# wei-zeng98/piano-a2s

Measured on AMD Instinct MI355X. Metric: training clips/sec (12 s, 5-bar), higher is better.
Workload: dtype f32

## Files before the change

include/a2s.h:

```cpp
#ifndef A2S_H
#define A2S_H
#include <stddef.h>
#include <stdint.h>
#ifdef __cplusplus
extern "C" {
#endif

#define A2S_OK 0
#define A2S_ERR_ARG (-1)
#define A2S_ERR_HIP (-2)
#define A2S_ERR_WORKSPACE (-3)

const char* a2s_last_error(void);
int a2s_version(void);
long long a2s_launch_count(void);

int a2s_gemm_f32(void* stream, int M, int N, int K, float alpha, const float* A, long sAm, long sAk,
                 const float* B, long sBk, long sBn, float beta, float* C, long ldc, const float* bias, int act,
                 int batch, long bsA, long bsB, long bsC, int splitk, float* workspace, size_t workspace_bytes);
int a2s_gemm_f32_affine(void* stream, int M, int N, int K, float alpha, const float* A, long sAm, long sAk, const float* B, long sBk,
                        long sBn, float beta, float* C, long ldc, const float* bias, int act, int batch, long bsA, long bsB, long bsC,
                        int splitk, float* workspace, size_t workspace_bytes, const float* a_scale, const float* a_shift, int a_period,
                        const float* b_scale, const float* b_shift, int b_period);
int a2s_gemm_f32_bnstats(void* stream, int M, int N, int K, const float* A, long sAm, long sAk, const float* B, long sBk, long sBn, float* C, long ldc,
// ... 7 lines not shown
                                const float* a_absmax, const float* b_absmax);
int a2s_linear_dgrad_bnstats(void* stream, int M, int N, int K, const float* dz, long lda, const float* Wt, float* da, long ldc, const float* y,
                             const float* mean, const float* invstd, const float* scale, const float* shift, int period, float* partial,
                             const float* dz_absmax, const float* w_absmax, float* workspace, size_t workspace_bytes, float* da_absmax_out);
int a2s_linear_fwd(void* stream, int M, int N, int K, const float* y, long lda, const float* W, float* z, long ldc, const float* scale, const float* shift,
                   int period, const float* y_absmax, const float* w_absmax, float* workspace, size_t workspace_bytes);
int a2s_linear_fwd_eligible(int M, int N, int K, int period);
int a2s_linear_wgrad(void* stream, int M, int N, int K, const float* dz, long ldz, const float* y, long lda, float* G, long ldg, const float* scale,
                     const float* shift, int period, const float* dz_absmax, const float* y_absmax, float* workspace, size_t workspace_bytes);
size_t a2s_linear_wgrad_ws_bytes(int M, int K);
int a2s_linear_wgrad_eligible(int M, int N, int K, int period);
int a2s_tallk_wgrad(void* stream, int M, int Np, int K, const float* P, long ldp, const float* A, long lda, float* G, long ldg, int transposed, float* bias,
                    const float* p_absmax, const float* a_absmax, float* workspace, size_t workspace_bytes);
size_t a2s_tallk_wgrad_ws_bytes(int M, int Np, int K);
int a2s_tallk_wgrad_eligible(int M, int Np, int K, long ldp, long lda, long ldg, int transposed);
size_t a2s_linear_dgrad_ws_bytes(int N, int K);
int a2s_linear_dgrad_blocks(int M);
int a2s_linear_dgrad_eligible(int M, int N, int K, int period);
int a2s_absmax(void* stream, const float* x, long n, float* out);
int a2s_gemm_bnstats_blocks(int M, int period);
size_t a2s_gemm_workspace_bytes(int M, int N, int batch, int splitk);
int a2s_gemm_pick_splitk(int M, int N, int K, int batch);
void a2s_gemm_debug_tile(int cfg);
int a2s_debug_set(const char* key, int value);
int a2s_debug_get(const char* key);
int a2s_env_check(void);
int a2s_persist_abort_latch(void* device_word);

int a2s_conv3x3(void* stream, const float* x, const float* w, float* y, const float* in_scale, const float* in_shift,
                float* stat_partial, int B, int T, int F, int Cin, int Cout, int flip, float* workspace);
// ... 323 lines not shown
```

piano_a2s_amd/csrc/a2s_api.hip:

```cpp
#define A2S_SWITCHES_IMPL
#include "a2s_internal.h"

thread_local char a2s_err_msg[512] = {0};
long long a2s_launch_counter = 0;

#define ST ((hipStream_t)stream)

extern "C" {

const char* a2s_last_error(void) { return a2s_err_msg; }
int a2s_version(void) { return 1; }
long long a2s_launch_count(void) { return __atomic_load_n(&a2s_launch_counter, __ATOMIC_RELAXED); }

int a2s_gemm_f32(void* stream, int M, int N, int K, float alpha, const float* A, long sAm, long sAk, const float* B, long sBk,
                 long sBn, float beta, float* C, long ldc, const float* bias, int act, int batch, long bsA, long bsB, long bsC,
                 int splitk, float* workspace, size_t workspace_bytes) {
    return a2s_gemm_impl(ST, M, N, K, alpha, A, sAm, sAk, B, sBk, sBn, beta, C, ldc, bias, act, batch, bsA, bsB, bsC, splitk,
                         workspace, workspace_bytes);
}
int a2s_gemm_f32_affine(void* stream, int M, int N, int K, float alpha, const float* A, long sAm, long sAk, const float* B, long sBk,
                        long sBn, float beta, float* C, long ldc, const float* bias, int act, int batch, long bsA, long bsB, long bsC,
                        int splitk, float* workspace, size_t workspace_bytes, const float* a_scale, const float* a_shift, int a_period,
                        const float* b_scale, const float* b_shift, int b_period) {
    return a2s_gemm_affine_impl(ST, M, N, K, alpha, A, sAm, sAk, B, sBk, sBn, beta, C, ldc, bias, act, batch, bsA, bsB, bsC, splitk,
// ... 27 lines not shown
    return a2s_linear_fwd_impl(ST, M, N, K, y, lda, W, z, ldc, scale, shift, period, y_absmax, w_absmax, workspace, workspace_bytes);
}
int a2s_linear_wgrad(void* stream, int M, int N, int K, const float* dz, long ldz, const float* y, long lda, float* G, long ldg, const float* scale,
                     const float* shift, int period, const float* dz_absmax, const float* y_absmax, float* workspace, size_t workspace_bytes) {
    return a2s_linear_wgrad_impl(ST, M, N, K, dz, ldz, y, lda, G, ldg, scale, shift, period, dz_absmax, y_absmax, workspace, workspace_bytes);
}
size_t a2s_linear_wgrad_ws_bytes(int M, int K) { return a2s_linear_wgrad_ws_bytes_impl(M, K); }
int a2s_linear_wgrad_eligible(int M, int N, int K, int period) { return a2s_linear_wgrad_ok(M, N, K, 256, 4, 4, period, nullptr, nullptr, nullptr) ? 1 : 0; }
int a2s_tallk_wgrad(void* stream, int M, int Np, int K, const float* P, long ldp, const float* A, long lda, float* G, long ldg, int transposed, float* bias,
                    const float* p_absmax, const float* a_absmax, float* workspace, size_t workspace_bytes) {
    return a2s_tallk_wgrad_impl(ST, M, Np, K, P, ldp, A, lda, G, ldg, transposed, bias, p_absmax, a_absmax, workspace, workspace_bytes);
}
size_t a2s_tallk_wgrad_ws_bytes(int M, int Np, int K) { return a2s_tallk_wgrad_ws_bytes_impl(M, Np, K); }
int a2s_tallk_wgrad_eligible(int M, int Np, int K, long ldp, long lda, long ldg, int transposed) {
    return a2s_tallk_wgrad_ok(M, Np, K, ldp, lda, ldg, transposed, nullptr, nullptr, nullptr, nullptr) ? 1 : 0;
}
int a2s_linear_fwd_eligible(int M, int N, int K, int period) { return a2s_linear_fwd_ok(M, N, K, 4, 4, period, nullptr, nullptr, nullptr) ? 1 : 0; }
int a2s_linear_dgrad_blocks(int M) { return a2s_linear_dgrad_blocks_impl(M); }
int a2s_linear_dgrad_eligible(int M, int N, int K, int period) {
    return a2s_linear_dgrad_ok(M, N, K, 4, 1, K, 4, period, nullptr, nullptr, nullptr, nullptr) ? 1 : 0;
}
int a2s_gemm_f32_bnstats(void* stream, int M, int N, int K, const float* A, long sAm, long sAk, const float* B, long sBk, long sBn, float* C, long ldc,
                         const float* y, const float* mean, const float* invstd, const float* scale, const float* shift, int period, float* partial) {
    return a2s_gemm_affine_impl(ST, M, N, K, 1.f, A, sAm, sAk, B, sBk, sBn, 0.f, C, ldc, nullptr, 0, 1, 0, 0, 0, 1, nullptr, 0,
                                nullptr, nullptr, 0, nullptr, nullptr, 0, y, mean, invstd, scale, shift, partial, period, 0, nullptr, nullptr);
}
int a2s_gemm_bnstats_blocks(int M, int period) { return a2s_cdiv(M, 128) * a2s_gemm_bnstats_slots(period); }
size_t a2s_gemm_workspace_bytes(int M, int N, int batch, int splitk) { return a2s_gemm_workspace_bytes_impl(M, N, batch, splitk); }
int a2s_gemm_pick_splitk(int M, int N, int K, int batch) { return a2s_gemm_pick_splitk_impl(M, N, K, batch); }
void a2s_gemm_debug_tile(int cfg) { a2s_gemm_debug_tile_impl(cfg); }
size_t a2s_note_step_workspace_floats(int H, int E) { return a2s_note_step_workspace_floats_impl(H, E); }
int a2s_debug_set(const char* key, int value) {
    if (!key) return A2S_ERR_ARG;
    const int id = a2s_switch_find(key);
    if (id >= 0) { a2s_switch_store(id, value); return A2S_OK; }
    if (!strcmp(key, "attn_deferred_fast")) { a2s_attn_deferred_fast = value ? 1 : 0; return A2S_OK; }
    if (!strcmp(key, "tallk_wgrad")) { a2s_tallk_wgrad_on = value ? 1 : 0; return A2S_OK; }
    if (!strcmp(key, "tallk_wgrad_max_splits")) { a2s_tallk_wgrad_max_splits = value > 0 ? value : 0; return A2S_OK; }
    if (!strcmp(key, "gemm_tile")) { a2s_gemm_debug_tile_impl(value); return A2S_OK; }
    snprintf(a2s_err_msg, sizeof(a2s_err_msg), "a2s_debug_set: unknown key %s", key);
    return A2S_ERR_ARG;
}
int a2s_env_check(void) {
    if (const char* e = a2s_switch_env_error()) A2S_FAIL(A2S_ERR_ARG, "%s: expected a decimal number >= 0", e);
    return A2S_OK;
}

int a2s_persist_abort_latch(void* device_word) { a2s_persist_latch_set(device_word); return A2S_OK; }

int a2s_debug_get(const char* key) {
    if (!key) return -1;
    const int id = a2s_switch_find(key);
    if (id == A2S_SW_attn_pair_fused_rows) return a2s_attn_pair_fused_rows();
    if (id >= 0) return a2s_sw((a2s_switch)id);
    if (!strcmp(key, "attn_pair_launches")) return (int)a2s_attn_pair_launches();
    if (!strcmp(key, "attn_pair_bwd_launches")) return (int)a2s_attn_pair_bwd_launches();
    if (!strcmp(key, "attn_deferred_fast")) return a2s_attn_deferred_fast;
    if (!strcmp(key, "tallk_wgrad")) return a2s_tallk_wgrad_on;
    if (!strcmp(key, "tallk_wgrad_max_splits")) return a2s_tallk_wgrad_max_splits;
    if (!strcmp(key, "tallk_wgrad_launches")) return (int)a2s_tallk_wgrad_launches();
    if (!strcmp(key, "attn_dk_ahead_launches")) return (int)a2s_attn_dk_ahead_launches();
    if (!strcmp(key, "attn_denc_launches")) return (int)a2s_attn_denc_launches();
    if (!strcmp(key, "dec_mid_launches")) return a2s_dec_mid_launches();
    if (!strcmp(key, "dec_cmb_launches")) return a2s_dec_cmb_launches();
    if (!strcmp(key, "dec_persist_launches")) return a2s_dec_persist_launches();
    if (!strcmp(key, "edit_distance_launches")) return (int)a2s_edit_distance_launches();
    if (!strcmp(key, "conv_rows16_c20_launches")) return (int)a2s_conv_rows16_c20_launches();
    if (!strcmp(key, "device_cus")) return a2s_device_geometry().cus;
    if (!strcmp(key, "device_xccs")) return a2s_device_geometry().xccs;
    return -1;
}

int a2s_conv3x3(void* stream, const float* x, const float* w, float* y, const float* in_scale, const float* in_shift,
                float* stat_partial, int B, int T, int F, int Cin, int Cout, int flip, float* workspace) {
    return a2s_conv3x3_impl(ST, x, w, y, in_scale, in_shift, stat_partial, B, T, F, Cin, Cout, flip, workspace, nullptr, nullptr, nullptr, nullptr, nullptr, nullptr,
// ... 411 lines not shown
```

piano_a2s_amd/csrc/a2s_bwd.hip:

```cpp
#include "a2s_internal.h"

__global__ __launch_bounds__(256) void log_softmax_bwd_rows(const float* __restrict__ g, const float* __restrict__ y,
                                                            long outer_stride, int inner, float* __restrict__ dx,
                                                            int R, int V, int n_outer, int time_major) {
    const int row = blockIdx.x * 4 + (threadIdx.x >> 6), lane = threadIdx.x & 63;
    if (row >= R) return;
    const int ob = row / inner, in = row % inner;
    const float* gr = g + (long)ob * outer_stride + (long)in * V;
    const float* yr = y + (long)ob * outer_stride + (long)in * V;
    float s = 0.f;
    for (int j = lane; j < V; j += 64) s += gr[j];
    s = wave_sum(s);
    const long orow = time_major ? ((long)in * n_outer + ob) : row;
    for (int j = lane; j < V; j += 64) dx[orow * V + j] = gr[j] - expf(yr[j]) * s;
}

int a2s_log_softmax_bwd_rows_impl(hipStream_t st, const float* g, const float* y, long outer_stride, int inner, float* dx,
                                  int R, int V, int n_outer, int time_major) {
    hipLaunchKernelGGL(log_softmax_bwd_rows, dim3(a2s_cdiv(R, 4)), dim3(256), 0, st, g, y, outer_stride, inner, dx, R, V, n_outer, time_major);
    A2S_CHECK_LAUNCH("log_softmax_bwd_rows");
    return A2S_OK;
}

__global__ void gru_gates_bwd(const float* __restrict__ dh_a, long lda, const float* __restrict__ dh_b, long ldb,
// ... 540 lines not shown
    if (idx >= rows * cols) return;
    const int c = idx / rows, r = idx % rows;
    out[idx] = in[(long)r * cols + c];
}

int a2s_gru_seq_bwd_impl(hipStream_t st, const float* dout, long do_bstride, long do_tstride, const float* out, long out_bstride,
                         long out_tstride, const float* gates, const float* w_hh, const float* dhn, float* dgi_all, float* dgh_shift,
                         float* dgh_first, float* dhbuf, float* dgh_tmp, int B, int T, int H, int reverse, float* ws, size_t ws_bytes,
                         float* ranges_out, int* ranges_valid) {
    A2S_REQUIRE(dout && out && gates && w_hh && dgi_all && dgh_shift && dgh_first && dhbuf && dgh_tmp, "gru_seq_bwd: null tensor");
    if (ranges_valid) *ranges_valid = 0;
    hipError_t e;
    if (dhn) e = hipMemcpyAsync(dhbuf, dhn, sizeof(float) * B * H, hipMemcpyDeviceToDevice, st);
    else e = hipMemsetAsync(dhbuf, 0, sizeof(float) * B * H, st);
    if (e != hipSuccess) A2S_FAIL(A2S_ERR_HIP, "gru_seq_bwd init: %s", hipGetErrorString(e));
    e = hipMemsetAsync(dgh_shift, 0, sizeof(float) * (size_t)B * T * 3 * H, st);
    if (e != hipSuccess) A2S_FAIL(A2S_ERR_HIP, "gru_seq_bwd memset: %s", hipGetErrorString(e));
    const bool fused = a2s_sw(A2S_SW_gru_fused) && H % 32 == 0 && ws && ws_bytes >= sizeof(float) * 3 * H * H && ((uintptr_t)ws % 16 == 0);
    if (fused) {
        hipLaunchKernelGGL(transpose_f32, dim3(a2s_cdiv(3 * H * H, 256)), dim3(256), 0, st, w_hh, ws, 3 * H, H);
        A2S_CHECK_LAUNCH("transpose_f32");
    }
    if (fused && a2s_gru_seq_bwd_persist_ok(B, T, H, ws, ws_bytes, sizeof(float) * 3 * (size_t)H * H)) {
        const int rc = a2s_gru_seq_bwd_persist_impl(st, dout, do_bstride, do_tstride, out, out_bstride, out_tstride, gates, ws, dhn, dgi_all, dgh_shift, dgh_first,
                                                    B, T, H, reverse, ws, sizeof(float) * 3 * (size_t)H * H, ws_bytes, ranges_out);
        if (rc == A2S_OK && ranges_out && ranges_valid) *ranges_valid = 1;
        return rc;
    }
    if (fused && ws_bytes >= sizeof(float) * (3 * (size_t)H * H + 3 * (size_t)B * H) && (3 * H * H) % 4 == 0) {
        float* tmp[2] = {dgh_tmp, ws + 3 * (size_t)H * H};
        auto tix = [&](int s) { return reverse ? T - 1 - s : s; };
// ... 895 lines not shown
```

piano_a2s_amd/csrc/a2s_internal.h:

```cpp
#pragma once
#include "a2s_common.h"
#include "../../include/a2s.h"
#include "a2s_switches.h"

static inline int a2s_attn_pair_fused_rows(void) {
    const int cap = a2s_sw(A2S_SW_dec_fused_max_rows), v = a2s_sw(A2S_SW_attn_pair_fused_rows);
    return v < cap ? v : cap;
}
static inline unsigned a2s_persist_dbg(void) {
    return (a2s_sw(A2S_SW_persist_force_agent) ? PERSIST_DBG_FORCE_AGENT : 0u) | (a2s_sw(A2S_SW_persist_inject_abort) ? PERSIST_DBG_INJECT_ABORT : 0u);
}

int a2s_absmax_impl(hipStream_t st, const float* x, long n, float* out);
size_t a2s_gemm_workspace_bytes_impl(int M, int N, int batch, int splitk);
int a2s_gemm_pick_splitk_impl(int M, int N, int K, int batch);
int a2s_gemm_bnstats_slots(int period);
void a2s_gemm_debug_tile_impl(int cfg);
int a2s_gemm_affine_impl(hipStream_t st, int M, int N, int K, float alpha, const float* A, long sAm, long sAk,
    const float* B, long sBk, long sBn, float beta, float* C, long ldc, const float* bias, int act,
    int batch, long bsA, long bsB, long bsC, int splitk, float* ws, size_t ws_bytes,
    const float* a_scale, const float* a_shift, int a_period, const float* b_scale, const float* b_shift, int b_period,
    const float* ep_y, const float* ep_mean, const float* ep_invstd, const float* ep_scale, const float* ep_shift,
    float* ep_partial, int ep_period, int two_term, const float* a_absmax, const float* b_absmax);
int a2s_gemm_impl(hipStream_t st, int M, int N, int K, float alpha, const float* A, long sAm, long sAk,
// ... 8 lines not shown
    float* partial, const float* a_absmax, const float* b_absmax, float* ws, size_t ws_bytes, float* c_absmax_out);
bool a2s_linear_fwd_ok(int M, int N, int K, long lda, long ldc, int period, const void* A, const void* W, const void* C);
int a2s_linear_fwd_impl(hipStream_t st, int M, int N, int K, const float* A, long lda, const float* W, float* C, long ldc, const float* a_scale,
    const float* a_shift, int period, const float* a_absmax, const float* w_absmax, float* ws, size_t ws_bytes);
size_t a2s_linear_wgrad_ws_bytes_impl(int M, int K);
bool a2s_linear_wgrad_ok(int M, int N, int K, long ldz, long lda, long ldg, int period, const void* dz, const void* A, const void* G);
int a2s_linear_wgrad_impl(hipStream_t st, int M, int N, int K, const float* dz, long ldz, const float* A, long lda, float* G, long ldg, const float* a_scale,
    const float* a_shift, int period, const float* dz_absmax, const float* a_absmax, float* ws, size_t ws_bytes);
extern int a2s_tallk_wgrad_on;
extern int a2s_tallk_wgrad_max_splits;
long a2s_tallk_wgrad_launches(void);
size_t a2s_tallk_wgrad_ws_bytes_impl(int M, int Np, int K);
bool a2s_tallk_wgrad_ok(int M, int Np, int K, long ldp, long lda, long ldg, int transposed, const void* P, const void* A, const void* G, const void* bias);
int a2s_tallk_wgrad_impl(hipStream_t st, int M, int Np, int K, const float* P, long ldp, const float* A, long lda, float* G, long ldg, int transposed,
    float* bias, const float* p_absmax, const float* a_absmax, float* ws, size_t ws_bytes);

int a2s_act_bound_impl(hipStream_t st, const float* scale, const float* shift, const float* absmax, int C, float* out);
size_t a2s_conv3x3_workspace_floats_impl(int Cin);
int a2s_conv3x3_impl(hipStream_t st, const float* x, const float* w, float* y, const float* in_scale,
    const float* in_shift, float* stat_partial, int B, int T, int F, int Cin, int Cout, int flip, float* ws,
    const float* yl, const float* yl_mean, const float* yl_invstd, const float* yl_scale, const float* yl_shift,
    const float* x_absmax, const float* in_absmax, float* out_absmax);
int a2s_conv3x3_stat_blocks_impl(int B, int T, int F, int Cin);
int a2s_bn_finalize_impl(hipStream_t st, const float* partial, int nblocks, int C, double count, const float* gamma,
    const float* beta, float* running_mean, float* running_var, long long* nbt, float* mean,
    float* invstd, float* scale, float* shift, float eps, float momentum, int training);
int a2s_bn_relu_apply_impl(hipStream_t st, const float* x, float* y, const float* scale, const float* shift, long n, int C, int F);
int a2s_col_stats_impl(hipStream_t st, const float* x, float* partial, long rows, int C, int rows_per_block);
int a2s_bn1d_relu_dropout_impl(hipStream_t st, const float* x, float* y, const float* scale, const float* shift,
    const uint8_t* mask, float inv_keep, long n, int C);
// ... 325 lines not shown
```

piano_a2s_amd/csrc/a2s_linear.hip:

```cpp
#include "a2s_internal.h"

#define LIN_BM 128
#define LIN_K 256
#define LIN_RS 288
#define LIN_NTH 512
#define LIN_LDS (2 * 2 * LIN_BM * LIN_RS)

typedef unsigned lu32x4 __attribute__((ext_vector_type(4)));

struct LinDgradArgs {
    const float* A; long lda;
    const unsigned char* planes;
    float* C; long ldc;
    const float* ep_y;
    const float* mean; const float* invstd; const float* scale; const float* shift;
    float* partial;
    const float* a_absmax; const float* b_absmax;
    int M, N, period, channels;
    float* c_absmax_out;
};

__global__ __launch_bounds__(256) void lin_pack_planes_k(const float* __restrict__ W, long ld, int N, int K, const float* __restrict__ absmax,
                                                         unsigned char* __restrict__ out) {
    const long id = (long)blockIdx.x * 256 + threadIdx.x;
// ... 646 lines not shown
    hipLaunchKernelGGL(lin_pack_dz_planes, dim3((unsigned)(((long)nsteps * 1024 + 255) / 256), npb), dim3(256), 0, st, P, ldp, M, nsteps, p_absmax, planes);
    A2S_CHECK_LAUNCH("lin_pack_dz_planes");
    LinWgradArgs a{A, lda, planes, partial, nullptr, nullptr, a_absmax, p_absmax, M, K, K, nblk, (nblk + splits - 1) / splits, (long)plane_stride, Np,
                   bias ? bias_partial : nullptr};
    if (bias) hipLaunchKernelGGL(lin_wgrad_roles<true>, dim3(K / LIN_BM, splits, npb), dim3(LIN_NTH), 0, st, a);
    else hipLaunchKernelGGL(lin_wgrad_roles<false>, dim3(K / LIN_BM, splits, npb), dim3(LIN_NTH), 0, st, a);
    A2S_CHECK_LAUNCH("lin_wgrad (tall-K)");
    const long n = (long)Np * K, nthreads = (n + (bias ? K : 0)) / 4;
    const dim3 rgrid((unsigned)((nthreads + 255) / 256));
    if (transposed) hipLaunchKernelGGL(lin_wgrad_reduce<true>, rgrid, dim3(256), 0, st, partial, splits, n, G, ldg, K, bias ? bias_partial : nullptr, bias);
    else hipLaunchKernelGGL(lin_wgrad_reduce<false>, rgrid, dim3(256), 0, st, partial, splits, n, G, ldg, K, bias ? bias_partial : nullptr, bias);
    A2S_CHECK_LAUNCH("lin_wgrad_reduce");
    __atomic_fetch_add(&g_tallk_launches, 1LL, __ATOMIC_RELAXED);
    return A2S_OK;
}
```

piano_a2s_amd/engine_bwd.py:

```python
import ctypes as C
import os
import threading
from collections import namedtuple

import torch

from . import hip
from .conv_bwd_plan import CHANS, ConvBwdFlags, plan_convstack_bwd
from .dec_bwd_plan import dim, plan_note_decoder_bwd, plan_staff_issue
from .spec import SOS, VOCAB_SIZE


def _ptr(t, off=0):
    return C.c_void_p(t.data_ptr() + 4 * off)


_COLSUM_WS = {}


def _colsum(x, ld, out, rows, ncol, x_off=0, out_off=0, beta=1.0):
    ws = None
    if rows >= 2048:
        key = (x.device, torch.cuda.current_stream().cuda_stream, threading.get_ident())
        ws = _COLSUM_WS.get(key)
# ... 362 lines not shown
            wg = _weight_grad_stream(dev)
            wg.wait_stream(torch.cuda.current_stream())
            with torch.cuda.stream(wg):
                for fn, ev, tensors in self.late:
                    wg.wait_event(ev)
                    for t in tensors:
                        if t is not None:
                            t.record_stream(wg)
                    fn()
            late_join = dec_lo
            self.late = []
        else:
            for gf in self.group_flat[1:]:
                flat.add_(gf)
        d_hid_carry = self.d_hidden
        if self.concurrent:
            dEnc.add_(self.dEnc_staff[0]).add_(self.dEnc_staff[1])
        enc2d = enc.view(B * T, H2)
        enc_amax = hip.absmax(enc)
        for p, dKp in dK.items():
            Wn = p + ".attn.attn.weight"
            dk_amax = hip.absmax(dKp)
            if not hip.tallk_wgrad(dKp, 0, H, enc2d, 0, H2, G[Wn], H2, 4 * H, B * T, H, H2, dk_amax, enc_amax):
                sk = L.a2s_gemm_pick_splitk(H, H2, B * T, 1)
                hip.gemm(dKp, 1, H, enc2d, H2, 1, G[Wn], 4 * H, H, H2, B * T, beta=1.0, splitk=sk, c_off=H2, two_term=(dk_amax, enc_amax))
            hip.gemm(dKp, H, 1, S[Wn], 4 * H, 1, dEnc, H2, B * T, H2, H, beta=1.0, b_off=H2, two_term=(dk_amax, hip.absmax(S[Wn])))
        if late_join is not None:
            wg = _weight_grad_stream(dev)
            wg.wait_stream(torch.cuda.current_stream())
            with torch.cuda.stream(wg):
                for gf in self.group_flat[1:]:
                    flat[late_join:].add_(gf[late_join:])
                if Backward.check_fold:
                    for gi, gf in enumerate(self.group_flat[1:], 1):
                        assert not bool(gf[:late_join].any()), f"clip group {gi}: non-decoder gradients in the group buffer would be lost by the late fold"
        d_conv = _encoder_bwd(eng, S, G, sv["enc"], dEnc, d_hid_carry, B, T)
        n_conv = next(off for k, off in zip(names, offs) if not k.startswith("convstack."))
        if grad_ready is not None:
            with torch.cuda.stream(_weight_grad_stream(dev)):
                grad_ready(self.flat_full, n_conv, total + 1)
        if getattr(eng, "conv_unperm", None) is not None:
# ... 71 lines not shown
            dgh_first, dhbuf, dgh_tmp = torch.empty((B, 3 * H), device=dev), torch.empty((2, B, H), device=dev), torch.empty((B, 3 * H), device=dev)
            ranges, valid = torch.empty(2, device=dev), C.c_int(0)
            if L.a2s_debug_get(b"tallk_wgrad") > 0:
                hip.check(L.a2s_gru_seq_bwd_ranged(hip.stream(), _ptr(dout, d * H), T * 2 * H, 2 * H, _ptr(out, d * H), T * 2 * H, 2 * H, hip._p(ls["dirs"][d]["gates"]),
                                                   hip._p(S[f"encoder.gru.weight_hh_{sfx}"]), hip._p(dhn[2 * layer + d]), hip._p(dgi), hip._p(dghs), hip._p(dgh_first),
                                                   hip._p(dhbuf), hip._p(dgh_tmp), B, T, H, d, hip._p(gws[d]), gws[d].numel() * 4, hip._p(ranges), C.byref(valid)),
                          "a2s_gru_seq_bwd_ranged")
            else:
                hip.check(L.a2s_gru_seq_bwd(hip.stream(), _ptr(dout, d * H), T * 2 * H, 2 * H, _ptr(out, d * H), T * 2 * H, 2 * H, hip._p(ls["dirs"][d]["gates"]),
                                            hip._p(S[f"encoder.gru.weight_hh_{sfx}"]), hip._p(dhn[2 * layer + d]), hip._p(dgi), hip._p(dghs), hip._p(dgh_first),
                                            hip._p(dhbuf), hip._p(dgh_tmp), B, T, H, d, hip._p(gws[d]), gws[d].numel() * 4), "a2s_gru_seq_bwd")
            return (dgi, dghs, dgh_first, dhbuf, dgh_tmp, ranges if valid.value else None)

        res = fork_on_streams(dev, streams, [lambda d=d, sfx=sfx: direction(d, sfx) for d, sfx in enumerate((f"l{layer}", f"l{layer}_reverse"))])()
        dgi_amax = []
        for d, sfx in enumerate((f"l{layer}", f"l{layer}_reverse")):
            dgi2 = res[d][0].view(B * T, 3 * H)
            Wih = S[f"encoder.gru.weight_ih_{sfx}"]
            ranges = res[d][5]
            tt = (ranges[0:1] if ranges is not None else hip.absmax(dgi2), hip.absmax(Wih))
            dgi_amax.append(tt[0])
            if L.a2s_debug_get(b"gemm_bf16x3") > 0:
                hip.gemm(dgi2, 3 * H, 1, Wih.t().contiguous(), 1, 3 * H, dX, I, B * T, I, 3 * H, beta=0.0 if d == 0 else 1.0, two_term=tt)
            else:
                hip.gemm(dgi2, 3 * H, 1, Wih, I, 1, dX, I, B * T, I, 3 * H, beta=0.0 if d == 0 else 1.0, two_term=tt)
        wg = _weight_grad_stream(dev)
        ev = torch.cuda.Event()
        ev.record()
        wg.wait_event(ev)
        for d, sfx in enumerate((f"l{layer}", f"l{layer}_reverse")):
            dgi, dghs, dgh_first, ranges = res[d][0], res[d][1], res[d][2], res[d][5]
            for t in (dgi, dghs, dgh_first, dgi_amax[d], in_amax, ranges):
                if t is not None:
                    t.record_stream(wg)
            with torch.cuda.stream(wg):
                dgi2, dghs2 = dgi.view(B * T, 3 * H), dghs.view(B * T, 3 * H)
# ... 99 lines not shown
```

piano_a2s_amd/hip.py:

```python
import ctypes as C
import os
import threading

import numpy as np
import torch

from .abi import PROTOTYPES, STRUCTS, A2SError
from .build import LIB

LIB = os.environ.get("A2S_LIB", LIB)

NoteDecArgs, NoteDecBwdArgs, BeamArgs, AlignArgs = (STRUCTS[n] for n in ("a2s_note_dec_args", "a2s_note_dec_bwd_args", "a2s_beam_args", "a2s_align_args"))
_lib = None


def set_row_plan(a, active):
    active = active or {}
    for field, key in (("clip_order", "order"), ("clip_rank", "rank"), ("row_until", "until"), ("row_list", "row_list")):
        setattr(a, field, active[key].data_ptr() if active.get(key) is not None else None)
    for field, key in (("n_active", "n_active"), ("m_active", "m_active"), ("n_rows_active", "n_rows_active")):
        host = active.get(key) if (key != "n_rows_active" or active.get("row_list") is not None) else None
        setattr(a, field, C.cast(host, C.c_void_p).value if host is not None else None)
    a.n_clips = active.get("n_clips", 0)

# ... 1126 lines not shown
        return False
    pp, pa, pg = P.data_ptr() + 4 * p_off, A.data_ptr() + 4 * a_off, G.data_ptr() + 4 * g_off
    if (p_absmax is None or a_absmax is None or (pp | pa | pg | (bias.data_ptr() if bias is not None else 0)) % 16
            or not L.a2s_tallk_wgrad_eligible(M, Np, K, ldp, lda, ldg, int(transposed))):
        return False
    nb = L.a2s_tallk_wgrad_ws_bytes(M, Np, K)
    key = (A.device, torch.cuda.current_stream().cuda_stream, threading.get_ident())
    ws = _TALLK_WS.get(key)
    if ws is None or ws.numel() * 4 < nb:
        ws = _TALLK_WS[key] = torch.empty((nb + 3) // 4, dtype=torch.float32, device=A.device)
    check(L.a2s_tallk_wgrad(stream(), M, Np, K, C.c_void_p(pp), ldp, C.c_void_p(pa), lda, C.c_void_p(pg), ldg, int(transposed), _p(bias), _p(p_absmax), _p(a_absmax),
                            _p(ws), ws.numel() * 4), "a2s_tallk_wgrad")
    return True


def linear_forward_for_test(x, w, aff):
    period = aff[2]
    xmax = x.view(x.shape[0], -1, period).abs().amax(dim=(0, 2)).contiguous()
    return linear_forward(x, w, aff, act_bound(aff[0], aff[1], xmax), absmax(w))
```

Before: 637.3.

## Fuse multi-segment data-gradient GEMMs and addend sums into one segmented kernel

Adds a segmented dgrad kernel that takes up to three (A, W) pairs along K into a single accumulator and folds up to three addend tensors into the epilogue. It uses split-f16 MFMA with warp-specialised loader waves. It replaces the separate per-key GEMMs plus elementwise adds for dEnc, and the two per-direction GRU input dgrad GEMMs for dX, cutting launches and read-modify-write passes over the output. The GRU backward memset is also narrowed to only the boundary timestep row. This adds a weight-packing launch on every call and a per-segment exponent rescale of the accumulators, which could affect precision.

```diff
diff --git a/include/a2s.h b/include/a2s.h
--- a/include/a2s.h
+++ b/include/a2s.h
@@ -45,6 +45,11 @@
                     const float* p_absmax, const float* a_absmax, float* workspace, size_t workspace_bytes);
 size_t a2s_tallk_wgrad_ws_bytes(int M, int Np, int K);
 int a2s_tallk_wgrad_eligible(int M, int Np, int K, long ldp, long lda, long ldg, int transposed);
+int a2s_seg_dgrad(void* stream, int M, int N, int nseg, const int* K, const float* const* A, const long* lda, const float* const* W, const long* sWk,
+                  const long* sWn, const float* const* a_absmax, const float* const* w_absmax, int nadd, const float* const* Cin, float* C, long ldc,
+                  float* workspace, size_t workspace_bytes);
+size_t a2s_seg_dgrad_ws_bytes(int N, int nseg, const int* K);
+int a2s_seg_dgrad_eligible(int M, int N, int nseg, const int* K, const long* lda, long ldc, int nadd);
 size_t a2s_linear_dgrad_ws_bytes(int N, int K);
 int a2s_linear_dgrad_blocks(int M);
 int a2s_linear_dgrad_eligible(int M, int N, int K, int period);
diff --git a/piano_a2s_amd/csrc/a2s_api.hip b/piano_a2s_amd/csrc/a2s_api.hip
--- a/piano_a2s_amd/csrc/a2s_api.hip
+++ b/piano_a2s_amd/csrc/a2s_api.hip
@@ -65,6 +65,15 @@
 size_t a2s_tallk_wgrad_ws_bytes(int M, int Np, int K) { return a2s_tallk_wgrad_ws_bytes_impl(M, Np, K); }
 int a2s_tallk_wgrad_eligible(int M, int Np, int K, long ldp, long lda, long ldg, int transposed) {
     return a2s_tallk_wgrad_ok(M, Np, K, ldp, lda, ldg, transposed, nullptr, nullptr, nullptr, nullptr) ? 1 : 0;
+}
+int a2s_seg_dgrad(void* stream, int M, int N, int nseg, const int* K, const float* const* A, const long* lda, const float* const* W, const long* sWk,
+                  const long* sWn, const float* const* a_absmax, const float* const* w_absmax, int nadd, const float* const* Cin, float* C, long ldc,
+                  float* workspace, size_t workspace_bytes) {
+    return a2s_seg_dgrad_impl(ST, M, N, nseg, K, A, lda, W, sWk, sWn, a_absmax, w_absmax, nadd, Cin, C, ldc, workspace, workspace_bytes);
+}
+size_t a2s_seg_dgrad_ws_bytes(int N, int nseg, const int* K) { return a2s_seg_dgrad_ws_bytes_impl(N, nseg, K); }
+int a2s_seg_dgrad_eligible(int M, int N, int nseg, const int* K, const long* lda, long ldc, int nadd) {
+    return a2s_seg_dgrad_ok(M, N, nseg, K, lda, ldc, nadd) ? 1 : 0;
 }
 int a2s_linear_fwd_eligible(int M, int N, int K, int period) { return a2s_linear_fwd_ok(M, N, K, 4, 4, period, nullptr, nullptr, nullptr) ? 1 : 0; }
 int a2s_linear_dgrad_blocks(int M) { return a2s_linear_dgrad_blocks_impl(M); }
@@ -88,6 +97,7 @@
     if (!strcmp(key, "attn_deferred_fast")) { a2s_attn_deferred_fast = value ? 1 : 0; return A2S_OK; }
     if (!strcmp(key, "tallk_wgrad")) { a2s_tallk_wgrad_on = value ? 1 : 0; return A2S_OK; }
     if (!strcmp(key, "tallk_wgrad_max_splits")) { a2s_tallk_wgrad_max_splits = value > 0 ? value : 0; return A2S_OK; }
+    if (!strcmp(key, "seg_dgrad")) { a2s_seg_dgrad_on = value ? 1 : 0; return A2S_OK; }
     if (!strcmp(key, "gemm_tile")) { a2s_gemm_debug_tile_impl(value); return A2S_OK; }
     snprintf(a2s_err_msg, sizeof(a2s_err_msg), "a2s_debug_set: unknown key %s", key);
     return A2S_ERR_ARG;
@@ -110,6 +120,8 @@
     if (!strcmp(key, "tallk_wgrad")) return a2s_tallk_wgrad_on;
     if (!strcmp(key, "tallk_wgrad_max_splits")) return a2s_tallk_wgrad_max_splits;
     if (!strcmp(key, "tallk_wgrad_launches")) return (int)a2s_tallk_wgrad_launches();
+    if (!strcmp(key, "seg_dgrad")) return a2s_seg_dgrad_on;
+    if (!strcmp(key, "seg_dgrad_launches")) return (int)a2s_seg_dgrad_launches();
     if (!strcmp(key, "attn_dk_ahead_launches")) return (int)a2s_attn_dk_ahead_launches();
     if (!strcmp(key, "attn_denc_launches")) return (int)a2s_attn_denc_launches();
     if (!strcmp(key, "dec_mid_launches")) return a2s_dec_mid_launches();
diff --git a/piano_a2s_amd/csrc/a2s_bwd.hip b/piano_a2s_amd/csrc/a2s_bwd.hip
--- a/piano_a2s_amd/csrc/a2s_bwd.hip
+++ b/piano_a2s_amd/csrc/a2s_bwd.hip
@@ -578,7 +578,7 @@
     if (dhn) e = hipMemcpyAsync(dhbuf, dhn, sizeof(float) * B * H, hipMemcpyDeviceToDevice, st);
     else e = hipMemsetAsync(dhbuf, 0, sizeof(float) * B * H, st);
     if (e != hipSuccess) A2S_FAIL(A2S_ERR_HIP, "gru_seq_bwd init: %s", hipGetErrorString(e));
-    e = hipMemsetAsync(dgh_shift, 0, sizeof(float) * (size_t)B * T * 3 * H, st);
+    e = hipMemset2DAsync(dgh_shift + (long)(reverse ? 0 : T - 1) * 3 * H, sizeof(float) * (size_t)T * 3 * H, 0, sizeof(float) * 3 * H, (size_t)B, st);
     if (e != hipSuccess) A2S_FAIL(A2S_ERR_HIP, "gru_seq_bwd memset: %s", hipGetErrorString(e));
     const bool fused = a2s_sw(A2S_SW_gru_fused) && H % 32 == 0 && ws && ws_bytes >= sizeof(float) * 3 * H * H && ((uintptr_t)ws % 16 == 0);
     if (fused) {
diff --git a/piano_a2s_amd/csrc/a2s_internal.h b/piano_a2s_amd/csrc/a2s_internal.h
--- a/piano_a2s_amd/csrc/a2s_internal.h
+++ b/piano_a2s_amd/csrc/a2s_internal.h
@@ -46,6 +46,13 @@
 bool a2s_tallk_wgrad_ok(int M, int Np, int K, long ldp, long lda, long ldg, int transposed, const void* P, const void* A, const void* G, const void* bias);
 int a2s_tallk_wgrad_impl(hipStream_t st, int M, int Np, int K, const float* P, long ldp, const float* A, long lda, float* G, long ldg, int transposed,
     float* bias, const float* p_absmax, const float* a_absmax, float* ws, size_t ws_bytes);
+extern int a2s_seg_dgrad_on;
+long a2s_seg_dgrad_launches(void);
+size_t a2s_seg_dgrad_ws_bytes_impl(int N, int nseg, const int* K);
+bool a2s_seg_dgrad_ok(int M, int N, int nseg, const int* K, const long* lda, long ldc, int nadd);
+int a2s_seg_dgrad_impl(hipStream_t st, int M, int N, int nseg, const int* K, const float* const* A, const long* lda, const float* const* W, const long* sWk,
+    const long* sWn, const float* const* a_absmax, const float* const* w_absmax, int nadd, const float* const* Cin, float* C, long ldc,
+    float* ws, size_t ws_bytes);
 
 int a2s_act_bound_impl(hipStream_t st, const float* scale, const float* shift, const float* absmax, int C, float* out);
 size_t a2s_conv3x3_workspace_floats_impl(int Cin);
diff --git a/piano_a2s_amd/csrc/a2s_linear.hip b/piano_a2s_amd/csrc/a2s_linear.hip
--- a/piano_a2s_amd/csrc/a2s_linear.hip
+++ b/piano_a2s_amd/csrc/a2s_linear.hip
@@ -684,3 +684,292 @@
     __atomic_fetch_add(&g_tallk_launches, 1LL, __ATOMIC_RELAXED);
     return A2S_OK;
 }
+
+#define LSEG_MAX 3
+struct LinSegArgs {
+    const float* A0; const float* A1; const float* A2; long lda0, lda1, lda2;
+    const unsigned char* pl0; const unsigned char* pl1; const unsigned char* pl2;
+    const float* aa0; const float* aa1; const float* aa2;
+    const float* ba0; const float* ba1; const float* ba2;
+    int nb0, nb1, nb2;
+    int e1, e2, nblk;
+    const float* Cin0; const float* Cin1; const float* Cin2;
+    float* C; long ldc;
+    int M, ncb, mtiles;
+};
+struct LinSegPack {
+    const float* W0; const float* W1; const float* W2; long sk0, sk1, sk2, sn0, sn1, sn2;
+    const float* am0; const float* am1; const float* am2;
+    unsigned char* o0; unsigned char* o1; unsigned char* o2;
+    int K0, K1, K2, N;
+};
+#define LSEG_SEL(s, x0, x1, x2) ((s) == 0 ? +(x0) : (s) == 1 ? +(x1) : +(x2))
+
+__global__ __launch_bounds__(256) void lin_pack_planes_seg(LinSegPack p) {
+    long id = (long)blockIdx.x * 256 + threadIdx.x;
+    int s = 0;
+    const long c0 = (long)(p.K0 >> 3) * p.N, c1 = (long)(p.K1 >> 3) * p.N, c2 = (long)(p.K2 >> 3) * p.N;
+    if (id >= c0) { id -= c0; s = 1; if (id >= c1) { id -= c1; s = 2; if (id >= c2) return; } }
+    const float* W = LSEG_SEL(s, p.W0, p.W1, p.W2);
+    const long sk = LSEG_SEL(s, p.sk0, p.sk1, p.sk2), sn = LSEG_SEL(s, p.sn0, p.sn1, p.sn2);
+    const int nks = LSEG_SEL(s, p.K0, p.K1, p.K2) >> 5;
+    unsigned char* out = LSEG_SEL(s, p.o0, p.o1, p.o2);
+    const int n = (int)(id % p.N), kg = (int)(id / p.N);
+    const float ps = ldexpf(1.f, pow2_scale_exp(*LSEG_SEL(s, p.am0, p.am1, p.am2), 12));
+    float x[8];
+#pragma unroll
+    for (int i = 0; i < 8; ++i) x[i] = __builtin_amdgcn_fmed3f(W[(long)(kg * 8 + i) * sk + (long)n * sn] * ps, -65000.f, 65000.f);
+    lu32x4 hi, lo;
+#pragma unroll
+    for (int i = 0; i < 4; ++i) { unsigned h, l; split2_pair_f16(x[2 * i], x[2 * i + 1], h, l); hi[i] = h; lo[i] = l; }
+    const int nt = n >> 4, lr = n & 15, ks = kg >> 2, lk = kg & 3;
+    unsigned char* o = out + ((((long)nt * nks + ks) * 2) * 64 + (lk * 16 + lr)) * 16;
+    *reinterpret_cast<lu32x4*>(o) = hi;
+    *reinterpret_cast<lu32x4*>(o + 64 * 16) = lo;
+}
+
+__global__ __launch_bounds__(LIN_NTH) void lin_seg_roles(LinSegArgs a) {
+    __shared__ __attribute__((aligned(16))) unsigned char lds[LF_NS * LF_STAGE];
+    const int tid = threadIdx.x, lane = tid & 63, lr = lane & 15, lk = lane >> 4;
+    const int wave = __builtin_amdgcn_readfirstlane(tid >> 6);
+    const int xcd = blockIdx.x & 7, slot = blockIdx.x >> 3;
+    const int cb = slot % a.ncb, tile = (slot / a.ncb) * 8 + xcd;
+    if (tile >= a.mtiles) return;
+    const int m0 = tile * LIN_BM;
+    const int e1 = a.e1, e2 = a.e2, nblk = a.nblk;
+#define LSEG_OF(blk) (((blk) >= e1 ? 1 : 0) + ((blk) >= e2 ? 1 : 0))
+    const int ka0 = pow2_scale_exp(*a.aa0, 12), ka1 = a.nb1 ? pow2_scale_exp(*a.aa1, 12) : 0, ka2 = a.nb2 ? pow2_scale_exp(*a.aa2, 12) : 0;
+    if (wave >= 4) {
+        const int st_ = tid - 256;
+        const int sk = (st_ & 15) * 4;
+        const float ps0 = ldexpf(1.f, ka0), ps1 = ldexpf(1.f, ka1), ps2 = ldexpf(1.f, ka2);
+        const bool stream_once = a.ncb == 1;
+        f32x4 ar[2][8];
+        auto issue_a = [&, e1, e2, nblk, st_, sk, stream_once](int blk, f32x4 (&r)[8]) {
+            const int s = LSEG_OF(blk);
+            const float* A = LSEG_SEL(s, a.A0, a.A1, a.A2);
+            const long lda = LSEG_SEL(s, a.lda0, a.lda1, a.lda2);
+            const int lb = blk - LSEG_SEL(s, 0, e1, e2);
+#pragma unroll
+            for (int i = 0; i < 8; ++i) {
+                const int row = (st_ + 256 * i) >> 4;
+                r[i] = (f32x4){0.f, 0.f, 0.f, 0.f};
+                if (m0 + row < a.M && blk < nblk) {
+                    const f32x4* src = reinterpret_cast<const f32x4*>(A + (long)(m0 + row) * lda + (long)lb * 64 + sk);
+                    r[i] = stream_once ? __builtin_nontemporal_load(src) : *src;
+                }
+            }
+        };
+        auto commit_a = [&, e1, e2, nblk, st_, sk, ps0, ps1, ps2](int blk, const f32x4 (&r)[8]) {
+            if (blk >= nblk) return;
+            const int s = LSEG_OF(blk);
+            float sc = LSEG_SEL(s, ps0, ps1, ps2);
+            if ((blk >> 2) & 1) sc = -sc;
+            unsigned char* st = lds + (blk % LF_NS) * LF_STAGE;
+#pragma unroll
+            for (int i = 0; i < 8; ++i) {
+                const int row = (st_ + 256 * i) >> 4;
+                float x[4];
+#pragma unroll
+                for (int j = 0; j < 4; ++j) x[j] = __builtin_amdgcn_fmed3f(r[i][j] * sc, -65000.f, 65000.f);
+                uint2 hi, lo;
+                split2_pair_f16(x[0], x[1], hi.x, lo.x);
+                split2_pair_f16(x[2], x[3], hi.y, lo.y);
+                *reinterpret_cast<uint2*>(st + (0 * LIN_BM + row) * LF_RS + sk * 2) = hi;
+                *reinterpret_cast<uint2*>(st + (1 * LIN_BM + row) * LF_RS + sk * 2) = lo;
+            }
+        };
+        issue_a(0, ar[0]);
+        commit_a(0, ar[0]);
+        issue_a(1, ar[1]); issue_a(2, ar[0]);
+#pragma unroll 1
+        for (int b0 = 0; b0 < nblk; b0 += 2) {
+            __syncthreads();
+            commit_a(b0 + 1, ar[1]); issue_a(b0 + 3, ar[1]);
+            if (b0 + 1 < nblk) {
+                __syncthreads();
+                commit_a(b0 + 2, ar[0]); issue_a(b0 + 4, ar[0]);
+            }
+        }
+        return;
+    }
+    const int kb0 = pow2_scale_exp(*a.ba0, 12), kb1 = a.nb1 ? pow2_scale_exp(*a.ba1, 12) : 0, kb2 = a.nb2 ? pow2_scale_exp(*a.ba2, 12) : 0;
+    const int ex0 = __builtin_amdgcn_readfirstlane(ka0 + kb0), ex1 = __builtin_amdgcn_readfirstlane(ka1 + kb1), ex2 = __builtin_amdgcn_readfirstlane(ka2 + kb2);
+    lu32x4 bf[2][4][2];
+    auto load_b = [&, e1, e2, nblk](int gks, lu32x4 (&dst)[4][2]) {
+        if (gks >= 2 * nblk) return;
+        const int s = LSEG_OF(gks >> 1);
+        const unsigned char* pl = LSEG_SEL(s, a.pl0, a.pl1, a.pl2);
+        const int nks = 2 * LSEG_SEL(s, a.nb0, a.nb1, a.nb2), ks = gks - 2 * LSEG_SEL(s, 0, e1, e2);
+#pragma unroll
+        for (int nt = 0; nt < 4; ++nt)
+#pragma unroll
+            for (int sp = 0; sp < 2; ++sp)
+                dst[nt][sp] = *reinterpret_cast<const lu32x4*>(pl + (((long)(cb * 16 + wave * 4 + nt) * nks + ks) * 2 + sp) * 1024 + (unsigned)lane * 16u);
+    };
+    f32x4 acc[8][4];
+#pragma unroll
+    for (int mt = 0; mt < 8; ++mt)
+#pragma unroll
+        for (int nt = 0; nt < 4; ++nt) acc[mt][nt] = (f32x4){0.f, 0.f, 0.f, 0.f};
+    load_b(0, bf[0]);
+    auto load_af = [&](const unsigned char* st, int h, int qt, lu32x4 (&af)[2][2]) {
+#pragma unroll
+        for (int sp = 0; sp < 2; ++sp)
+#pragma unroll
+            for (int q = 0; q < 2; ++q) af[sp][q] = *reinterpret_cast<const lu32x4*>(st + (sp * LIN_BM + (qt * 2 + q) * 16 + lr) * LF_RS + h * 64 + lk * 16);
+    };
+    auto multiply = [&](int qt, const lu32x4 (&af)[2][2], const lu32x4 (&b)[4][2]) {
+#define LS_PRODUCT(SA, SB)                                                                                                        \
+        _Pragma("unroll") for (int nt = 0; nt < 4; ++nt)                                                                          \
+            _Pragma("unroll") for (int q = 0; q < 2; ++q)                                                                         \
+                acc[qt * 2 + q][nt] = __builtin_amdgcn_mfma_f32_16x16x32_f16(__builtin_bit_cast(f16x8, b[nt][SB]),                \
+                                                                             __builtin_bit_cast(f16x8, af[SA][q]), acc[qt * 2 + q][nt], 0, 0, 0);
+        LS_PRODUCT(1, 0) LS_PRODUCT(0, 1) LS_PRODUCT(0, 0)
+#undef LS_PRODUCT
+    };
+    int cur_ex = ex0;
+    bool neg = false;
+#pragma unroll 1
+    for (int blk = 0; blk < nblk; ++blk) {
+        const int want_ex = LSEG_SEL(LSEG_OF(blk), ex0, ex1, ex2);
+        const bool want = (blk >> 2) & 1;
+        if (want_ex != cur_ex || want != neg) {
+            const int d = want_ex - cur_ex;
+            const float sg = want != neg ? -1.f : 1.f;
+#pragma unroll
+            for (int mt = 0; mt < 8; ++mt)
+#pragma unroll
+                for (int nt = 0; nt < 4; ++nt)
+#pragma unroll
+                    for (int r = 0; r < 4; ++r) acc[mt][nt][r] = ldexpf(acc[mt][nt][r] * sg, d);
+            cur_ex = want_ex; neg = want;
+        }
+        __syncthreads();
+        const unsigned char* st = lds + (blk % LF_NS) * LF_STAGE;
+        lu32x4 fa[2][2], fb[2][2];
+        load_af(st, 0, 0, fa);
+        load_b(2 * blk + 1, bf[1]);
+        __builtin_amdgcn_sched_barrier(0);
+        load_af(st, 0, 1, fb); multiply(0, fa, bf[0]);
+        __builtin_amdgcn_sched_barrier(0);
+        load_af(st, 0, 2, fa); multiply(1, fb, bf[0]);
+        __builtin_amdgcn_sched_barrier(0);
+        load_af(st, 0, 3, fb); multiply(2, fa, bf[0]);
+        __builtin_amdgcn_sched_barrier(0);
+        load_af(st, 1, 0, fa); multiply(3, fb, bf[0]);
+        __builtin_amdgcn_sched_barrier(0);
+        load_b(2 * blk + 2, bf[0]);
+        load_af(st, 1, 1, fb); multiply(0, fa, bf[1]);
+        __builtin_amdgcn_sched_barrier(0);
+        load_af(st, 1, 2, fa); multiply(1, fb, bf[1]);
+        __builtin_amdgcn_sched_barrier(0);
+        load_af(st, 1, 3, fb); multiply(2, fa, bf[1]);
+        __builtin_amdgcn_sched_barrier(0);
+        multiply(3, fb, bf[1]);
+        __builtin_amdgcn_sched_barrier(0);
+    }
+    const float sg = neg ? -1.f : 1.f;
+    const long col = (long)cb * 256 + wave * 64 + lk * 4;
+    const bool h0 = a.Cin0 != nullptr, h1 = a.Cin1 != nullptr, h2 = a.Cin2 != nullptr;
+#pragma unroll
+    for (int mp = 0; mp < 4; ++mp) {
+        f32x4 add[2][4];
+#pragma unroll
+        for (int u = 0; u < 2; ++u) {
+            const int m = m0 + (mp * 2 + u) * 16 + lr;
+#pragma unroll
+            for (int nt = 0; nt < 4; ++nt) {
+                const long off = (long)m * a.ldc + col + nt * 16;
+                f32x4 s = (f32x4){0.f, 0.f, 0.f, 0.f};
+                if (m < a.M) {
+                    if (h0) s = *reinterpret_cast<const f32x4*>(a.Cin0 + off);
+                    if (h1) { const f32x4 t = *reinterpret_cast<const f32x4*>(a.Cin1 + off); for (int r = 0; r < 4; ++r) s[r] += t[r]; }
+                    if (h2) { const f32x4 t = *reinterpret_cast<const f32x4*>(a.Cin2 + off); for (int r = 0; r < 4; ++r) s[r] += t[r]; }
+                }
+                add[u][nt] = s;
+            }
+        }
+#pragma unroll
+        for (int u = 0; u < 2; ++u) {
+            const int mt = mp * 2 + u, m = m0 + mt * 16 + lr;
+            if (m >= a.M) continue;
+#pragma unroll
+            for (int nt = 0; nt < 4; ++nt) {
+                f32x4 v;
+#pragma unroll
+                for (int r = 0; r < 4; ++r) v[r] = ldexpf(acc[mt][nt][r] * sg, -cur_ex) + add[u][nt][r];
+                *reinterpret_cast<f32x4*>(a.C + (long)m * a.ldc + col + nt * 16) = v;
+            }
+        }
+    }
+}
+
+#undef LSEG_OF
+#undef LSEG_SEL
+
+int a2s_seg_dgrad_on = 1;
+static long long g_seg_dgrad_launches = 0;
+long a2s_seg_dgrad_launches(void) { return (long)__atomic_load_n(&g_seg_dgrad_launches, __ATOMIC_RELAXED); }
+
+size_t a2s_seg_dgrad_ws_bytes_impl(int N, int nseg, const int* K) {
+    if ((N != 256 && N != 512) || nseg < 1 || nseg > LSEG_MAX || !K) return 0;
+    size_t n = 0;
+    for (int s = 0; s < nseg; ++s) {
+        if (K[s] < 64 || K[s] % 64 || K[s] > (1 << 20)) return 0;
+        n += (size_t)N * K[s] * 2 * 2;
+    }
+    return n;
+}
+bool a2s_seg_dgrad_ok(int M, int N, int nseg, const int* K, const long* lda, long ldc, int nadd) {
+    if (!a2s_seg_dgrad_on || M < 1 || M > (1 << 30) - LIN_BM || !lda || nadd < 0 || nadd > 3 || ldc < N || ldc % 4) return false;
+    if (!a2s_seg_dgrad_ws_bytes_impl(N, nseg, K)) return false;
+    for (int s = 0; s < nseg; ++s)
+        if (lda[s] < K[s] || lda[s] % 4) return false;
+    return true;
+}
+int a2s_seg_dgrad_impl(hipStream_t st, int M, int N, int nseg, const int* K, const float* const* A, const long* lda, const float* const* W, const long* sWk,
+                       const long* sWn, const float* const* a_absmax, const float* const* w_absmax, int nadd, const float* const* Cin, float* C, long ldc,
+                       float* ws, size_t ws_bytes) {
+    A2S_REQUIRE(K && A && lda && W && sWk && sWn && a_absmax && w_absmax && C && ws && (nadd == 0 || Cin), "seg_dgrad: null argument");
+    A2S_REQUIRE(a2s_seg_dgrad_ok(M, N, nseg, K, lda, ldc, nadd),
+                "seg_dgrad: needs N = 256 or 512, 1-3 segments with K %% 64 == 0, 0-3 addends, lda %% 4 == 0, ldc %% 4 == 0 (or the switch \"seg_dgrad\" is off)");
+    uintptr_t al = (uintptr_t)C | (uintptr_t)ws;
+    for (int s = 0; s < nseg; ++s) {
+        A2S_REQUIRE(A[s] && W[s] && a_absmax[s] && w_absmax[s], "seg_dgrad: null argument in segment %d", s);
+        al |= (uintptr_t)A[s];
+    }
+    for (int j = 0; j < nadd; ++j) {
+        A2S_REQUIRE(Cin[j], "seg_dgrad: null addend %d", j);
+        al |= (uintptr_t)Cin[j];
+    }
+    A2S_REQUIRE(al % 16 == 0, "seg_dgrad: operands, addends, result and workspace must be 16-byte aligned");
+    const size_t need = a2s_seg_dgrad_ws_bytes_impl(N, nseg, K);
+    A2S_REQUIRE(ws_bytes >= need, "seg_dgrad: workspace too small (%zu bytes needed)", need);
+    unsigned char* pl[LSEG_MAX] = {nullptr, nullptr, nullptr};
+    const float* Av[LSEG_MAX] = {nullptr, nullptr, nullptr};
+    const float* Wv[LSEG_MAX] = {nullptr, nullptr, nullptr};
+    const float* aav[LSEG_MAX] = {nullptr, nullptr, nullptr};
+    const float* bav[LSEG_MAX] = {nullptr, nullptr, nullptr};
+    const float* cin[3] = {nullptr, nullptr, nullptr};
+    long ldav[LSEG_MAX] = {0, 0, 0}, skv[LSEG_MAX] = {0, 0, 0}, snv[LSEG_MAX] = {0, 0, 0};
+    int Kv[LSEG_MAX] = {0, 0, 0};
+    unsigned char* next = reinterpret_cast<unsigned char*>(ws);
+    long pack_threads = 0;
+    for (int s = 0; s < nseg; ++s) {
+        pl[s] = next; next += (size_t)N * K[s] * 4;
+        Av[s] = A[s]; Wv[s] = W[s]; aav[s] = a_absmax[s]; bav[s] = w_absmax[s]; ldav[s] = lda[s]; skv[s] = sWk[s]; snv[s] = sWn[s]; Kv[s] = K[s];
+        pack_threads += (long)(K[s] / 8) * N;
+    }
+    for (int j = 0; j < nadd; ++j) cin[j] = Cin[j];
+    LinSegPack p{Wv[0], Wv[1], Wv[2], skv[0], skv[1], skv[2], snv[0], snv[1], snv[2], bav[0], bav[1], bav[2], pl[0], pl[1], pl[2], Kv[0], Kv[1], Kv[2], N};
+    hipLaunchKernelGGL(lin_pack_planes_seg, dim3((unsigned)((pack_threads + 255) / 256)), dim3(256), 0, st, p);
+    A2S_CHECK_LAUNCH("lin_pack_planes_seg");
+    const int mtiles = (M + LIN_BM - 1) / LIN_BM, ncb = N / 256;
+    LinSegArgs a{Av[0], Av[1], Av[2], ldav[0], ldav[1], ldav[2], pl[0], pl[1], pl[2], aav[0], aav[1], aav[2], bav[0], bav[1], bav[2],
+                 Kv[0] / 64, Kv[1] / 64, Kv[2] / 64, Kv[0] / 64, (Kv[0] + Kv[1]) / 64, (Kv[0] + Kv[1] + Kv[2]) / 64, cin[0], cin[1], cin[2], C, ldc, M, ncb, mtiles};
+    hipLaunchKernelGGL(lin_seg_roles, dim3((unsigned)(((mtiles + 7) / 8) * 8 * ncb)), dim3(LIN_NTH), 0, st, a);
+    A2S_CHECK_LAUNCH("lin_seg_roles");
+    __atomic_fetch_add(&g_seg_dgrad_launches, 1LL, __ATOMIC_RELAXED);
+    return A2S_OK;
+}
diff --git a/piano_a2s_amd/engine_bwd.py b/piano_a2s_amd/engine_bwd.py
--- a/piano_a2s_amd/engine_bwd.py
+++ b/piano_a2s_amd/engine_bwd.py
@@ -400,17 +400,22 @@
             for gf in self.group_flat[1:]:
                 flat.add_(gf)
         d_hid_carry = self.d_hidden
-        if self.concurrent:
-            dEnc.add_(self.dEnc_staff[0]).add_(self.dEnc_staff[1])
         enc2d = enc.view(B * T, H2)
         enc_amax = hip.absmax(enc)
+        key_segs = []
         for p, dKp in dK.items():
             Wn = p + ".attn.attn.weight"
             dk_amax = hip.absmax(dKp)
             if not hip.tallk_wgrad(dKp, 0, H, enc2d, 0, H2, G[Wn], H2, 4 * H, B * T, H, H2, dk_amax, enc_amax):
                 sk = L.a2s_gemm_pick_splitk(H, H2, B * T, 1)
                 hip.gemm(dKp, 1, H, enc2d, H2, 1, G[Wn], 4 * H, H, H2, B * T, beta=1.0, splitk=sk, c_off=H2, two_term=(dk_amax, enc_amax))
-            hip.gemm(dKp, H, 1, S[Wn], 4 * H, 1, dEnc, H2, B * T, H2, H, beta=1.0, b_off=H2, two_term=(dk_amax, hip.absmax(S[Wn])))
+            key_segs.append((dKp, 0, H, H, S[Wn], H2, 4 * H, 1, dk_amax, hip.absmax(S[Wn])))
+        staff = list(self.dEnc_staff) if self.concurrent else []
+        if not hip.seg_dgrad(key_segs, [dEnc] + staff, dEnc, H2, B * T, H2):
+            for t in staff:
+                dEnc.add_(t)
+            for dKp, _, _, _, Wp, _, _, _, dk_amax, w_amax in key_segs:
+                hip.gemm(dKp, H, 1, Wp, 4 * H, 1, dEnc, H2, B * T, H2, H, beta=1.0, b_off=H2, two_term=(dk_amax, w_amax))
         if late_join is not None:
             wg = _weight_grad_stream(dev)
             wg.wait_stream(torch.cuda.current_stream())
@@ -512,12 +517,16 @@
 
         res = fork_on_streams(dev, streams, [lambda d=d, sfx=sfx: direction(d, sfx) for d, sfx in enumerate((f"l{layer}", f"l{layer}_reverse"))])()
         dgi_amax = []
+        dx_segs = []
         for d, sfx in enumerate((f"l{layer}", f"l{layer}_reverse")):
             dgi2 = res[d][0].view(B * T, 3 * H)
             Wih = S[f"encoder.gru.weight_ih_{sfx}"]
             ranges = res[d][5]
             tt = (ranges[0:1] if ranges is not None else hip.absmax(dgi2), hip.absmax(Wih))
             dgi_amax.append(tt[0])
+            dx_segs.append((dgi2, 0, 3 * H, 3 * H, Wih, 0, I, 1, tt[0], tt[1]))
+        for d, seg in enumerate([] if hip.seg_dgrad(dx_segs, [], dX, I, B * T, I) else dx_segs):
+            dgi2, Wih, tt = seg[0], seg[4], seg[8:10]
             if L.a2s_debug_get(b"gemm_bf16x3") > 0:
                 hip.gemm(dgi2, 3 * H, 1, Wih.t().contiguous(), 1, 3 * H, dX, I, B * T, I, 3 * H, beta=0.0 if d == 0 else 1.0, two_term=tt)
             else:
diff --git a/piano_a2s_amd/hip.py b/piano_a2s_amd/hip.py
--- a/piano_a2s_amd/hip.py
+++ b/piano_a2s_amd/hip.py
@@ -1164,6 +1164,34 @@
     return True
 
 
+_SEG_WS = {}
+
+
+def seg_dgrad(segments, addends, Cout, ldc, M, N):
+    L = lib()
+    ns, na = len(segments), len(addends)
+    if not hasattr(L, "a2s_seg_dgrad_eligible") or not 1 <= ns <= 3 or na > 3:
+        return False
+    Ks = (C.c_int * ns)(*[s[3] for s in segments])
+    ldas = (C.c_long * ns)(*[s[2] for s in segments])
+    pa = [s[0].data_ptr() + 4 * s[1] for s in segments]
+    pw = [s[4].data_ptr() + 4 * s[5] for s in segments]
+    pc = [t.data_ptr() for t in addends]
+    if (any(s[8] is None or s[9] is None for s in segments) or any(p % 16 for p in pa + pw + pc + [Cout.data_ptr()])
+            or not L.a2s_seg_dgrad_eligible(M, N, ns, Ks, ldas, ldc, na)):
+        return False
+    nb = L.a2s_seg_dgrad_ws_bytes(N, ns, Ks)
+    key = (Cout.device, torch.cuda.current_stream().cuda_stream, threading.get_ident())
+    ws = _SEG_WS.get(key)
+    if ws is None or ws.numel() * 4 < nb:
+        ws = _SEG_WS[key] = torch.empty((nb + 3) // 4, dtype=torch.float32, device=Cout.device)
+    ptrs = lambda v: (C.c_void_p * max(len(v), 1))(*v)
+    check(L.a2s_seg_dgrad(stream(), M, N, ns, Ks, ptrs(pa), ldas, ptrs(pw), (C.c_long * ns)(*[s[6] for s in segments]), (C.c_long * ns)(*[s[7] for s in segments]),
+                          ptrs([s[8].data_ptr() for s in segments]), ptrs([s[9].data_ptr() for s in segments]), na, ptrs(pc), _p(Cout), ldc, _p(ws), ws.numel() * 4),
+          "a2s_seg_dgrad")
+    return True
+
+
 def linear_forward_for_test(x, w, aff):
     period = aff[2]
     xmax = x.view(x.shape[0], -1, period).abs().amax(dim=(0, 2)).contiguous()
```

Result: no change. 641.3 (median of 6 runs) (+0.6%).
